# CPJKU/audio_sheet_retrieval

Hardware: AMD Instinct MI355X
Metric: snippet-pairs/sec embedded+ranked (32-d CCA) (higher is better)
Workload: dtype f32

## Files before the change

### audio_sheet_retrieval_amd/csrc/conv_wino4_kernels.hip

```cpp
#include <hip/hip_runtime.h>
#include <stdint.h>
#include <stdlib.h>
#include <algorithm>
#include <type_traits>
#include <vector>
#include "asr_kernels.h"
#include "repack_elems.inl"

#ifndef ASR_WINO4_ABL
#define ASR_WINO4_ABL 0
#endif

namespace asr {

typedef float floatx4q __attribute__((ext_vector_type(4)));
typedef float float2q __attribute__((ext_vector_type(2)));

struct Wino4Args {
    const float *in, *wpk, *bnp;
    float *out;
    int N, H, W, OH, OW;
    int ty_img, tx_img;
    int coutp;
    int tiles;
    int total;
    double *stats;
    BnBwdFuse bf;
};

__device__ __forceinline__ float elu_fastq(float y) { return y > 0.0f ? y : __expf(y) - 1.0f; }

template <typename T> __device__ __forceinline__ T splatq(float c);
template <> __device__ __forceinline__ float2q splatq<float2q>(float c) { return float2q{c, c}; }
template <> __device__ __forceinline__ floatx4q splatq<floatx4q>(float c) { return floatx4q{c, c, c, c}; }
template <typename T> __device__ __forceinline__ T fmaq(float c, T x, T y) {
    return __builtin_elementwise_fma(splatq<T>(c), x, y);
}

template <typename T> __device__ __forceinline__ void in6(T &d0, T &d1, T &d2, T &d3, T &d4, T &d5) {
    const T r0 = fmaq(4.f, d0, fmaq(-5.f, d2, d4));
    const T t1 = fmaq(-4.f, d2, d4), t2 = fmaq(-4.f, d1, d3);
    const T t3 = d4 - d2, t4 = d3 - d1;
    const T r5 = fmaq(4.f, d1, fmaq(-5.f, d3, d5));
    d0 = r0; d1 = t1 + t2; d2 = t1 - t2; d3 = fmaq(2.f, t4, t3); d4 = fmaq(-2.f, t4, t3); d5 = r5;
}
template <typename T> __device__ __forceinline__ void out6(T m0, T m1, T m2, T m3, T m4, T m5, T &y0, T &y1, T &y2, T &y3) {
    const T s1 = m1 + m2, s2 = m1 - m2, s3 = m3 + m4, s4 = m3 - m4;
    y0 = (m0 + s1) + s3;
    y1 = fmaq(2.f, s4, s2);
    y2 = fmaq(4.f, s3, s1);
    y3 = fmaq(8.f, s4, s2) + m5;
}

template <int CIN, int COUT, bool POOL, int WAVES, bool RAW>
__global__ __launch_bounds__(64 * WAVES, 1) void conv3x3_wino4g(Wino4Args a) {
    constexpr int KS = CIN / 4, NB = CIN / 8, T = 64 * WAVES;
    constexpr int WS = 16;
    constexpr int WD = 6;
    constexpr int WQ = 72;
    static_assert(CIN % 8 == 0, "channel blocks of 8");
    extern __shared__ __align__(16) float w_lds[];
    const int tid = threadIdx.x, lane = tid & 63;
    const int wave = __builtin_amdgcn_readfirstlane(tid >> 6);
    const int nt0 = blockIdx.y;
    for (int i = tid; i < KS * 36 * 4 * 16; i += T) {
        const int row = i >> 4, nn = i & 15;
        const int gg = row & 3, kp = row >> 2, ks = kp / 36, p = kp - ks * 36;
        const int qq = (ks & 1) * 36 + p;
        w_lds[i] = a.wpk[((((size_t)(ks >> 1) * 18 + (qq >> 2)) * 4 + gg) * a.coutp + nt0 * 16 + nn) * 4 + (qq & 3)];
    }
    __syncthreads();

    const int m = lane & 15, g = lane >> 4, n = lane & 15;
    const float *w_lane = w_lds + g * WS + n;
    const int chn = nt0 * 16 + n;
    const bool ch_ok = chn < COUT;
    const float bmean = (!RAW && ch_ok) ? a.bnp[chn] : 0.f;
    const float bscale = (!RAW && ch_ok) ? a.bnp[a.coutp + chn] : 1.f;
    const float bbeta = (!RAW && ch_ok) ? a.bnp[2 * a.coutp + chn] : 0.f;
    const int per_img = a.ty_img * a.tx_img;

    for (int mt = blockIdx.x * WAVES + wave; mt < a.total; mt += gridDim.x * WAVES) {
        const int tnum = mt * 16 + m;
        const bool tvalid = tnum < a.tiles;
        const int tcl = min(tnum, a.tiles - 1);
        const int img = tcl / per_img;
        const int trest = tcl - img * per_img;
        const int tty = trest / a.tx_img, ttx = trest - tty * a.tx_img;
        const int py = 4 * tty, px = 4 * ttx;
        const float *ibase = a.in + (int64_t)img * a.H * a.W * CIN + 2 * g;
        int rowb[6], colb[6];
        unsigned oy_m = 0, ox_m = 0;
#pragma unroll
        for (int i = 0; i < 6; ++i) {
            const int y = py - 1 + i, x = px - 1 + i;
            oy_m |= (unsigned)(y >= 0 && y < a.H) << i;
            ox_m |= (unsigned)(x >= 0 && x < a.W) << i;
            rowb[i] = min(max(y, 0), a.H - 1) * a.W * CIN;
            colb[i] = min(max(x, 0), a.W - 1) * CIN;
        }
        if (!tvalid) oy_m = 0;
        const bool interior = __builtin_amdgcn_ballot_w64(oy_m != 0x3fu || ox_m != 0x3fu) == 0;
        unsigned my_off;
        int my_ext;
        if (POOL) {
            my_off = (((unsigned)img * a.OH + 2 * tty) * a.OW + 2 * ttx) * COUT;
            const int nr = min(2, a.OH - 2 * tty), nc = min(2, a.OW - 2 * ttx);
            my_ext = (tvalid && nr > 0 && nc > 0) ? (nr | (nc << 8)) : 0;
        } else {
            my_off = (((unsigned)img * a.H + py) * a.W + px) * COUT;
            const int nr = min(4, a.H - py), nc = min(4, a.W - px);
            my_ext = tvalid ? (nr | (nc << 8)) : 0;
        }

        floatx4q acc[36];
#pragma unroll
        for (int p = 0; p < 36; ++p) acc[p] = floatx4q{0.f, 0.f, 0.f, 0.f};

        float2q nxt[6][6];
#pragma unroll
        for (int i = 0; i < 6; ++i)
#pragma unroll
            for (int j = 0; j < 6; ++j) nxt[i][j] = *reinterpret_cast<const float2q *>(ibase + rowb[i] + colb[j]);
        float wpre[WD];
#pragma unroll
        for (int q = 0; q < WD; ++q) wpre[q] = w_lane[q * 4 * WS];
#pragma unroll 1
        for (int t = 0; t < NB; ++t) {
            float2q dp[6][6];
            if (interior) {
#pragma unroll
                for (int i = 0; i < 6; ++i)
#pragma unroll
                    for (int j = 0; j < 6; ++j) dp[i][j] = nxt[i][j];
            } else {
#pragma unroll
                for (int i = 0; i < 6; ++i)
#pragma unroll
                    for (int j = 0; j < 6; ++j)
                        dp[i][j] = (((oy_m >> i) & (ox_m >> j)) & 1u) ? nxt[i][j] : float2q{0.f, 0.f};
            }
            if (t + 1 < NB && !(ASR_WINO4_ABL & 2)) {
#pragma unroll
                for (int i = 0; i < 6; ++i)
#pragma unroll
                    for (int j = 0; j < 6; ++j)
                        nxt[i][j] = *reinterpret_cast<const float2q *>(ibase + rowb[i] + colb[j] + 8 * (t + 1));
            }
#pragma unroll
            for (int j = 0; j < 6; ++j) in6(dp[0][j], dp[1][j], dp[2][j], dp[3][j], dp[4][j], dp[5][j]);
#pragma unroll
            for (int i = 0; i < 6; ++i) in6(dp[i][0], dp[i][1], dp[i][2], dp[i][3], dp[i][4], dp[i][5]);
            const float *wk = w_lane + (2 * t) * (36 * 4 * WS);
            const float *wn = (t + 1 < NB) ? wk + 2 * 36 * 4 * WS : w_lane;
            float wv[WQ + WD];
#pragma unroll
            for (int q = 0; q < WD; ++q) wv[q] = wpre[q];
#pragma unroll
            for (int q0 = 0; q0 < WQ; q0 += 2) {
#pragma unroll
                for (int q = q0; q < q0 + 2; ++q)
                    wv[q + WD] = (q + WD < WQ) ? wk[(q + WD) * 4 * WS] : wn[(q + WD - WQ) * 4 * WS];
                __builtin_amdgcn_sched_barrier(0);
#pragma unroll
                for (int q = q0; q < q0 + 2; ++q) {
                    const int c = q / 36, p = q % 36;
                    acc[p] = __builtin_amdgcn_mfma_f32_16x16x4f32(dp[p / 6][p % 6][c], wv[q], acc[p], 0, 0, 0);
                }
                __builtin_amdgcn_sched_barrier(0);
            }
#pragma unroll
            for (int q = 0; q < WD; ++q) wpre[q] = wv[WQ + q];
        }

        unsigned eo[4];
        int ee[4];
#pragma unroll
        for (int r = 0; r < 4; ++r) {
            eo[r] = (unsigned)__shfl((int)my_off, 4 * g + r);
            ee[r] = __shfl(my_ext, 4 * g + r);
        }
        if (!ch_ok) continue;
        floatx4q tc[4][6];
#pragma unroll
        for (int nu = 0; nu < 6; ++nu)
            out6(acc[nu], acc[6 + nu], acc[12 + nu], acc[18 + nu], acc[24 + nu], acc[30 + nu], tc[0][nu], tc[1][nu], tc[2][nu],
                 tc[3][nu]);
        if (POOL) {
#pragma unroll
            for (int pr = 0; pr < 2; ++pr) {
                floatx4q ya[4], yb[4];
                out6(tc[2 * pr][0], tc[2 * pr][1], tc[2 * pr][2], tc[2 * pr][3], tc[2 * pr][4], tc[2 * pr][5], ya[0], ya[1],
                     ya[2], ya[3]);
                out6(tc[2 * pr + 1][0], tc[2 * pr + 1][1], tc[2 * pr + 1][2], tc[2 * pr + 1][3], tc[2 * pr + 1][4],
                     tc[2 * pr + 1][5], yb[0], yb[1], yb[2], yb[3]);
#pragma unroll
                for (int pc = 0; pc < 2; ++pc) {
#pragma unroll
                    for (int r = 0; r < 4; ++r) {
                        if (pr >= (ee[r] & 0xff) || pc >= (ee[r] >> 8)) continue;
                        const float v0 = ya[2 * pc][r], v1 = ya[2 * pc + 1][r], v2 = yb[2 * pc][r], v3 = yb[2 * pc + 1][r];
                        const float hi = fmaxf(fmaxf(v0, v1), fmaxf(v2, v3));
                        const float lo = fminf(fminf(v0, v1), fminf(v2, v3));
                        const float x = bscale >= 0.0f ? hi : lo;
                        a.out[(size_t)eo[r] + (size_t)(pr * a.OW + pc) * COUT + chn] =
                            elu_fastq((x - bmean) * bscale + bbeta);
                    }
                }
            }
        } else {
#pragma unroll
            for (int i = 0; i < 4; ++i) {
                floatx4q y[4];
                out6(tc[i][0], tc[i][1], tc[i][2], tc[i][3], tc[i][4], tc[i][5], y[0], y[1], y[2], y[3]);
#pragma unroll
                for (int j = 0; j < 4; ++j) {
#pragma unroll
                    for (int r = 0; r < 4; ++r) {
                        if (i >= (ee[r] & 0xff) || j >= (ee[r] >> 8)) continue;
                        const float v = RAW ? y[j][r] : elu_fastq((y[j][r] - bmean) * bscale + bbeta);
                        a.out[(size_t)eo[r] + (size_t)(i * a.W + j) * COUT + chn] = v;
                    }
                }
            }
        }
    }
}

template <int CIN, int COUT, bool POOL, int SLICE = COUT, int PW = 1, bool RAW = false>
__global__ __launch_bounds__(64 * (PW + (SLICE + 15) / 16), 1) void conv3x3_wino4s(Wino4Args a) {
    static_assert(!(RAW && POOL), "the raw form has no pooled epilogue");
    constexpr int NT = (SLICE + 15) / 16, NB = CIN / 8, KS = CIN / 4;
    static_assert(PW == 1 || PW == 2, "one or two producer waves");
    static_assert(PW + NT <= 4, "one wave per SIMD");
    static_assert(SLICE == COUT || (SLICE % 16 == 0 && COUT % SLICE == 0), "slices are whole n-tiles");
    constexpr int VB = 36 * 16 * 8;
    static_assert(CIN % 8 == 0, "channel blocks of 8");
    extern __shared__ __align__(16) float vbuf[];
    const int tid = threadIdx.x, lane = tid & 63;
    const int wave = __builtin_amdgcn_readfirstlane(tid >> 6);
    const bool producer = wave < PW;
    const int m = lane & 15, g = lane >> 4, n = lane & 15;
    const int per_img = a.ty_img * a.tx_img;

    int mt, mt_end, mt_stride;
    if ((gridDim.x & 7) == 0) {
        const int per_x = (a.total + 7) >> 3;
        const int r0 = (int)(blockIdx.x & 7) * per_x;
        mt_end = min(r0 + per_x, a.total);
        mt_stride = (int)(gridDim.x >> 3);
        mt = r0 + (int)(blockIdx.x >> 3);
    } else {
        mt_end = a.total; mt_stride = (int)gridDim.x; mt = (int)blockIdx.x;
    }
    if (mt >= mt_end) {
        if constexpr (RAW) {
            if (a.stats)
                for (int c = threadIdx.x; c < 2 * COUT; c += blockDim.x) a.stats[(size_t)blockIdx.x * 2 * COUT + c] = 0.0;
        }
        return;
    }

    auto tile_of = [&](int mtile, int &img, int &tty, int &ttx, bool &tvalid) {
        const int tnum = mtile * 16 + m;
        tvalid = tnum < a.tiles;
        const int tcl = min(tnum, a.tiles - 1);
        img = tcl / per_img;
        const int trest = tcl - img * per_img;
        tty = trest / a.tx_img;
        ttx = trest - tty * a.tx_img;
    };
    float *vlane = vbuf + (g * 32 + 2 * m);
#ifdef ASR_WINO4_OLD_V
    vlane = vbuf + (m * 8 + 2 * g);
#endif

    if (producer) {
        unsigned poff[6][6];
        unsigned oy_m = 0, ox_m = 0;
        auto setup = [&](int mtile) {
            int img, tty, ttx;
            bool tvalid;
            tile_of(mtile, img, tty, ttx, tvalid);
            const int py = 4 * tty, px = 4 * ttx;
            const unsigned ib = ((unsigned)img * a.H * a.W * CIN + 2 * g) * 4u;
            unsigned rowb[6], colb[6];
            oy_m = 0; ox_m = 0;
#pragma unroll
            for (int i = 0; i < 6; ++i) {
                const int y = py - 1 + i, x = px - 1 + i;
                oy_m |= (unsigned)(y >= 0 && y < a.H) << i;
                ox_m |= (unsigned)(x >= 0 && x < a.W) << i;
                rowb[i] = (unsigned)(min(max(y, 0), a.H - 1) * a.W * CIN) * 4u;
                colb[i] = (unsigned)(min(max(x, 0), a.W - 1) * CIN) * 4u;
            }
            if (!tvalid) oy_m = 0;
#pragma unroll
            for (int i = 0; i < 6; ++i)
#pragma unroll
                for (int j = 0; j < 6; ++j) poff[i][j] = ib + rowb[i] + colb[j];
        };
        float2q nxt[6][6];
        auto load = [&](int t) {
            const char *cb = reinterpret_cast<const char *>(a.in + 8 * t);
#pragma unroll
            for (int i = 0; i < 6; ++i)
#pragma unroll
                for (int j = 0; j < 6; ++j) nxt[i][j] = *reinterpret_cast<const float2q *>(cb + poff[i][j]);
        };
        const int n_mt = (mt_end - mt + mt_stride - 1) / mt_stride;
        const int n_steps = n_mt * NB;
        int passed = 0;
        int t = wave;
        while (t >= NB) { t -= NB; mt += mt_stride; }
        if (mt < mt_end) { setup(mt); load(t); }
        for (int step = wave; step < n_steps; step += PW) {
            float2q dp[6][6];
            const unsigned oy = oy_m, ox = ox_m;
            const bool interior = __builtin_amdgcn_ballot_w64(oy != 0x3fu || ox != 0x3fu) == 0;
            if (interior) {
#pragma unroll
                for (int i = 0; i < 6; ++i)
#pragma unroll
                    for (int j = 0; j < 6; ++j) dp[i][j] = nxt[i][j];
            } else {
#pragma unroll
                for (int i = 0; i < 6; ++i)
#pragma unroll
                    for (int j = 0; j < 6; ++j) dp[i][j] = (((oy >> i) & (ox >> j)) & 1u) ? nxt[i][j] : float2q{0.f, 0.f};
            }
            {
                int tn = t + PW, mtn = mt;
                while (tn >= NB) { tn -= NB; mtn += mt_stride; }
                if (!(ASR_WINO4_ABL & 2) && step + PW < n_steps) {
                    if (mtn != mt) setup(mtn);
                    load(tn);
                }
                t = tn; mt = mtn;
            }
            if (!(ASR_WINO4_ABL & 8)) {
#pragma unroll
            for (int j = 0; j < 6; ++j) in6(dp[0][j], dp[1][j], dp[2][j], dp[3][j], dp[4][j], dp[5][j]);
#pragma unroll
            for (int i = 0; i < 6; ++i) in6(dp[i][0], dp[i][1], dp[i][2], dp[i][3], dp[i][4], dp[i][5]);
            }
            while (passed < step) { __syncthreads(); ++passed; }
            float *vb = vlane + (step & 1) * VB;
            if (!(ASR_WINO4_ABL & 16)) {
#pragma unroll
            for (int p = 0; p < 36; ++p) *reinterpret_cast<float2q *>(vb + p * 128) = dp[p / 6][p % 6];
            } else {
#pragma unroll
            for (int p = 0; p < 36; ++p) asm volatile("" ::"v"(dp[p / 6][p % 6]));
            }
            __syncthreads();
            ++passed;
        }
        while (passed < n_steps + 1) { __syncthreads(); ++passed; }
        return;
    }

    const int nt = wave - PW;
    const int chn = (int)blockIdx.y * SLICE + nt * 16 + n;
    const bool ch_ok = chn < COUT;
    float bmean = (!RAW && ch_ok) ? a.bnp[chn] : 0.f;
    float bscale = (!RAW && ch_ok) ? a.bnp[a.coutp + chn] : 1.f;
    float bbeta = (!RAW && ch_ok) ? a.bnp[2 * a.coutp + chn] : 0.f;
    float bistd = 0.f;
    const bool bnb = ASR_BNB_FUSE_BUILD && RAW && a.stats && a.bf.z != nullptr;
    if (bnb && ch_ok) {
        bmean = a.bf.cst[chn]; bistd = a.bf.cst[COUT + chn];
        bscale = a.bf.cst[2 * COUT + chn]; bbeta = a.bf.cst[3 * COUT + chn];
    }
    double st1 = 0.0, st2 = 0.0;
    const unsigned wlane = ((unsigned)g * a.coutp + chn) * 16u;
    const float *wl = a.wpk;
    constexpr int wstep = 4 * ((COUT + 15) / 16 * 16);
    floatx4q bw[2][18];
#pragma unroll
    for (int j = 0; j < 18; ++j)
        bw[0][j] = *reinterpret_cast<const floatx4q *>(reinterpret_cast<const char *>(wl) + (size_t)j * (wstep * 16) + wlane);
    int step = 0;
    for (; mt < mt_end; mt += mt_stride) {
        unsigned my_off;
        int my_ext;
        {
            int img, tty, ttx;
            bool tvalid;
            tile_of(mt, img, tty, ttx, tvalid);
            if (POOL) {
                my_off = (((unsigned)img * a.OH + 2 * tty) * a.OW + 2 * ttx) * COUT;
                const int nr = min(2, a.OH - 2 * tty), nc = min(2, a.OW - 2 * ttx);
                my_ext = (tvalid && nr > 0 && nc > 0) ? (nr | (nc << 8)) : 0;
            } else {
                my_off = (((unsigned)img * a.H + 4 * tty) * a.W + 4 * ttx) * COUT;
                const int nr = min(4, a.H - 4 * tty), nc = min(4, a.W - 4 * ttx);
                my_ext = tvalid ? (nr | (nc << 8)) : 0;
            }
        }
        unsigned voff[9];
#pragma unroll
        for (int k = 0; k < 9; ++k) {
            voff[k] = wlane + (unsigned)k * (2 * wstep * 16);
            asm volatile("" : "+v"(voff[k]));
        }
        floatx4q acc[36];
        auto reload = [&](const float *wn, auto set_c) {
            constexpr int SET = decltype(set_c)::value;
            if (ASR_WINO4_ABL & 4) return;
            const char *wnb = reinterpret_cast<const char *>(wn);
#pragma unroll
            for (int k = 0; k < 9; ++k) {
                unsigned vo = voff[k];
                asm volatile("" : "+v"(vo));
                bw[SET][2 * k] = *reinterpret_cast<const floatx4q *>(wnb + vo);
                bw[SET][2 * k + 1] = *reinterpret_cast<const floatx4q *>(wnb + (wstep * 16) + vo);
            }
        };
        auto run_step = [&](const float *vb, const float *wn, auto cur_c, auto first) {
            constexpr bool FIRST = decltype(first)::value;
            constexpr int CUR = decltype(cur_c)::value;
            using NXT = std::integral_constant<int, CUR ^ 1>;
            __syncthreads();
            reload(wn, NXT{});
            __builtin_amdgcn_sched_barrier(0);
            float2q dp[2][12];
#pragma unroll
            for (int i = 0; i < 12; ++i) dp[0][i] = *reinterpret_cast<const float2q *>(vb + i * 128);
#pragma unroll
            for (int grp = 0; grp < 3; ++grp) {
                if (grp < 2) {
#pragma unroll
                    for (int i = 0; i < 12; ++i)
                        dp[(grp + 1) & 1][i] = *reinterpret_cast<const float2q *>(vb + ((grp + 1) * 12 + i) * 128);
                }
#pragma unroll
                for (int c = 0; c < 2; ++c)
#pragma unroll
                    for (int i = 0; i < 12; ++i) {
                        const int p = grp * 12 + i;
                        if (FIRST && c == 0)
                            acc[p] = __builtin_amdgcn_mfma_f32_16x16x4f32(dp[grp & 1][i][c], bw[CUR][(c * 36 + p) >> 2][(c * 36 + p) & 3],
                                                                          floatx4q{0.f, 0.f, 0.f, 0.f}, 0, 0, 0);
                        else
                            acc[p] = __builtin_amdgcn_mfma_f32_16x16x4f32(dp[grp & 1][i][c], bw[CUR][(c * 36 + p) >> 2][(c * 36 + p) & 3], acc[p],
                                                                          0, 0,
                                                                          0);
                    }
                __builtin_amdgcn_sched_barrier(0);
            }
        };
        using C0 = std::integral_constant<int, 0>;
        using C1 = std::integral_constant<int, 1>;
        auto wblock = [&](int t) {
            unsigned blk = (unsigned)(((t + 1) % NB) * 72) * wstep;
            asm volatile("" : "+s"(blk));
            return wl + blk;
        };
        run_step(vlane + (step & 1) * VB, wblock(0), C0{}, std::true_type{});
        ++step;
#pragma unroll 1
        for (int t = 1; t + 1 < NB; t += 2) {
            run_step(vlane + (step & 1) * VB, wblock(t), C1{}, std::false_type{});
            ++step;
            run_step(vlane + (step & 1) * VB, wblock(t + 1), C0{}, std::false_type{});
            ++step;
        }
        if constexpr ((NB & 1) == 0) {
            run_step(vlane + (step & 1) * VB, wblock(NB - 1), C1{}, std::false_type{});
            ++step;
        } else {
#pragma unroll
            for (int j = 0; j < 18; ++j) bw[0][j] = bw[1][j];
        }

        unsigned eo[4];
        int ee[4];
#pragma unroll
        for (int r = 0; r < 4; ++r) {
            eo[r] = (unsigned)__shfl((int)my_off, 4 * g + r);
            ee[r] = __shfl(my_ext, 4 * g + r);
        }
        if (!ch_ok) continue;
        floatx4q tc[4][6];
#pragma unroll
        for (int nu = 0; nu < 6; ++nu)
            out6(acc[nu], acc[6 + nu], acc[12 + nu], acc[18 + nu], acc[24 + nu], acc[30 + nu], tc[0][nu], tc[1][nu], tc[2][nu],
                 tc[3][nu]);
        if (POOL) {
#pragma unroll
            for (int pr = 0; pr < 2; ++pr) {
                floatx4q ya[4], yb[4];
                out6(tc[2 * pr][0], tc[2 * pr][1], tc[2 * pr][2], tc[2 * pr][3], tc[2 * pr][4], tc[2 * pr][5], ya[0], ya[1],
                     ya[2], ya[3]);
                out6(tc[2 * pr + 1][0], tc[2 * pr + 1][1], tc[2 * pr + 1][2], tc[2 * pr + 1][3], tc[2 * pr + 1][4],
                     tc[2 * pr + 1][5], yb[0], yb[1], yb[2], yb[3]);
#pragma unroll
                for (int pc = 0; pc < 2; ++pc) {
#pragma unroll
                    for (int r = 0; r < 4; ++r) {
                        if (pr >= (ee[r] & 0xff) || pc >= (ee[r] >> 8)) continue;
                        const float v0 = ya[2 * pc][r], v1 = ya[2 * pc + 1][r], v2 = yb[2 * pc][r], v3 = yb[2 * pc + 1][r];
                        const float hi = fmaxf(fmaxf(v0, v1), fmaxf(v2, v3));
                        const float lo = fminf(fminf(v0, v1), fminf(v2, v3));
                        const float x = bscale >= 0.0f ? hi : lo;
                        const float res = elu_fastq((x - bmean) * bscale + bbeta);
                        if (ASR_WINO4_ABL & 32) asm volatile("" ::"v"(res));
                        else a.out[(size_t)eo[r] + (size_t)(pr * a.OW + pc) * COUT + chn] = res;
                    }
                }
            }
        } else {
#pragma unroll
            for (int i = 0; i < 4; ++i) {
                floatx4q y[4];
                out6(tc[i][0], tc[i][1], tc[i][2], tc[i][3], tc[i][4], tc[i][5], y[0], y[1], y[2], y[3]);
                float rs1 = 0.f, rs2 = 0.f;
#pragma unroll
                for (int j = 0; j < 4; ++j) {
#pragma unroll
                    for (int r = 0; r < 4; ++r) {
                        if (i >= (ee[r] & 0xff) || j >= (ee[r] >> 8)) continue;
                        const float res = RAW ? y[j][r] : elu_fastq((y[j][r] - bmean) * bscale + bbeta);
                        if (RAW) {
                            if (bnb) {
                                const size_t e = (size_t)eo[r] + (size_t)(i * a.W + j) * COUT + chn;
                                bnb_acc(res, a.bf.z[e], bnb_mult(a.bf.tie, e), bmean, bscale, bbeta, bistd, rs1, rs2);
                            } else { rs1 += res; rs2 = fmaf(res, res, rs2); }
                        }
                        if (ASR_WINO4_ABL & 32) asm volatile("" ::"v"(res));
                        else a.out[(size_t)eo[r] + (size_t)(i * a.W + j) * COUT + chn] = res;
                    }
                }
                if (RAW) { st1 += (double)rs1; st2 += (double)rs2; }
            }
        }
    }
    __syncthreads();
    if constexpr (RAW) {
        if (a.stats) {
            st1 += __shfl_xor(st1, 16); st2 += __shfl_xor(st2, 16);
            st1 += __shfl_xor(st1, 32); st2 += __shfl_xor(st2, 32);
            if (g == 0 && ch_ok) {
                a.stats[((size_t)blockIdx.x * 2) * COUT + chn] = st1;
                a.stats[((size_t)blockIdx.x * 2 + 1) * COUT + chn] = st2;
            }
        }
    }
}

__global__ void wino4_pack_kernel(const float *W, int cin, int cout, int dgrad, float *wpk) {
    const int idx = blockIdx.x * blockDim.x + threadIdx.x;
    if (idx >= wino4_pack_count(cin, cout, dgrad)) return;
    wino4_pack_elem(idx, W, cin, cout, dgrad, wpk);
}

size_t wino4_wpack_floats(int cin, int cout) { return (cin % 8) ? 0 : (size_t)36 * cin * ((cout + 15) / 16 * 16); }

hipError_t launch_wino4_pack(hipStream_t s, const float *W, int cin, int cout, float *wpk, int dgrad) {
    const int kdim = dgrad ? cout : cin, ndim = dgrad ? cin : cout;
    if (kdim % 8) return hipSuccess;
    const int total = kdim * ((ndim + 15) / 16 * 16);
    hipLaunchKernelGGL(wino4_pack_kernel, dim3((total + 255) / 256), dim3(256), 0, s, W, cin, cout, dgrad, wpk);
    return hipGetLastError();
}

struct Wino4Variant {
    int cin, cout, pool, waves, raw;
    void (*kernel)(Wino4Args);
    const char *symbol;
    int spec;
    int slice;
};
#define ASR_BOOLSTRQ_0 "false"
#define ASR_BOOLSTRQ_1 "true"
#define ASR_WINO4(CIN, COUT, POOL, WAVES)                                                                         \
    { CIN, COUT, POOL, WAVES, 0, conv3x3_wino4g<CIN, COUT, (POOL != 0), WAVES, false>,                            \
      "void asr::conv3x3_wino4g<" #CIN ", " #COUT ", " ASR_BOOLSTRQ_##POOL ", " #WAVES ", false>(asr::Wino4Args)" }
#define ASR_WINO4S(CIN, COUT, POOL)                                                                               \
    { CIN, COUT, POOL, 1 + (COUT + 15) / 16, 0, conv3x3_wino4s<CIN, COUT, (POOL != 0)>,                           \
      "void asr::conv3x3_wino4s<" #CIN ", " #COUT ", " ASR_BOOLSTRQ_##POOL ", " #COUT ", 1, false>(asr::Wino4Args)", 1, 0 }
#define ASR_WINO4S2(CIN, COUT, POOL)                                                                              \
    { CIN, COUT, POOL, 2 + (COUT + 15) / 16, 0, conv3x3_wino4s<CIN, COUT, (POOL != 0), COUT, 2>,                  \
      "void asr::conv3x3_wino4s<" #CIN ", " #COUT ", " ASR_BOOLSTRQ_##POOL ", " #COUT ", 2, false>(asr::Wino4Args)", 1, 0 }
#define ASR_WINO4SR(CIN, COUT)                                                                                    \
    { CIN, COUT, 0, 1 + (COUT + 15) / 16, 1, conv3x3_wino4s<CIN, COUT, false, COUT, 1, true>,                     \
      "void asr::conv3x3_wino4s<" #CIN ", " #COUT ", false, " #COUT ", 1, true>(asr::Wino4Args)", 1, 0 }
#define ASR_WINO4SL(CIN, COUT, POOL, SLICE)                                                                       \
    { CIN, COUT, POOL, 1 + SLICE / 16, 0, conv3x3_wino4s<CIN, COUT, (POOL != 0), SLICE>,                          \
      "void asr::conv3x3_wino4s<" #CIN ", " #COUT ", " ASR_BOOLSTRQ_##POOL ", " #SLICE ", 1, false>(asr::Wino4Args)", 1, SLICE }
static const Wino4Variant g_wino4[] = {
    ASR_WINO4(24, 24, 1, 4), ASR_WINO4(24, 48, 0, 4), ASR_WINO4(48, 48, 1, 4), ASR_WINO4(48, 48, 0, 4),
    ASR_WINO4S(24, 24, 1), ASR_WINO4S(24, 48, 0), ASR_WINO4S(48, 48, 1), ASR_WINO4S(48, 48, 0),
    ASR_WINO4S2(24, 24, 1),
    ASR_WINO4SL(48, 96, 0, 48), ASR_WINO4SL(96, 96, 1, 48), ASR_WINO4SL(96, 96, 0, 48),
    ASR_WINO4SR(24, 48), ASR_WINO4SR(48, 48), ASR_WINO4SR(48, 24),
};
static const int g_num_wino4 = (int)(sizeof(g_wino4) / sizeof(g_wino4[0]));

void conv_candidates_wino4(int cin, int cout, int pool, int H, int W, std::vector<ConvPlan> *out) {
    static const int use = getenv("ASR_CONV_WINO4") ? atoi(getenv("ASR_CONV_WINO4")) : -1;
    if (use == 0) return;
    for (int vi = 0; vi < g_num_wino4; ++vi) {
        const Wino4Variant &v = g_wino4[vi];
        if (v.cin != cin || v.cout != cout || v.pool != pool || v.raw) continue;
        if (!v.spec && use != 1) continue;
        const int lds = v.spec ? 2 * 36 * 16 * 8 * 4 : 36 * cin * 16 * 4;
        (void)hipFuncSetAttribute(reinterpret_cast<const void *>(v.kernel), hipFuncAttributeMaxDynamicSharedMemorySize,
                                  160 * 1024);
        int nb = 0;
        if (hipOccupancyMaxActiveBlocksPerMultiprocessor(&nb, reinterpret_cast<const void *>(v.kernel), 64 * v.waves,
                                                         (size_t)lds) != hipSuccess || nb < 1) {
            (void)hipGetLastError();
            nb = 1;
        }
        ConvPlan bp{};
        bp.cin = cin; bp.cout = cout; bp.pool = pool;
        bp.H = H; bp.W = W; bp.OH = pool ? H / 2 : H; bp.OW = pool ? W / 2 : W;
        bp.TH = 4; bp.TW = 64; bp.NI = 16;
        bp.tiles_y = (H + 3) / 4; bp.tiles_x = (W + 3) / 4;
        bp.threads = 64 * v.waves;
        bp.lds_bytes = lds;
        bp.blocks_per_cu = v.spec ? 1 : std::min(nb, 4);
        bp.cost = (double)bp.tiles_y * bp.tiles_x / 16.0 * ((cout + 15) / 16) * (36.0 * (cin / 4) * 32.0 + 3000.0) *
                  (v.spec ? 0.4 : 1.0);
        bp.variant = 4000 + vi;
        bp.symbol = v.symbol;
        out->push_back(bp);
    }
}

void conv_candidates_wino4_raw(int cin, int cout, int H, int W, std::vector<ConvPlan> *out, int dgrad) {
    static const int use = getenv("ASR_TRAIN_WINO4") ? atoi(getenv("ASR_TRAIN_WINO4")) : -1;
    if (use == 0 || (use == 5 && !dgrad)) return;
    for (int vi = 0; vi < g_num_wino4; ++vi) {
        const Wino4Variant &v = g_wino4[vi];
        if (v.cin != cin || v.cout != cout || !v.raw) continue;
        const int lds = 2 * 36 * 16 * 8 * 4;
        (void)hipFuncSetAttribute(reinterpret_cast<const void *>(v.kernel), hipFuncAttributeMaxDynamicSharedMemorySize,
                                  160 * 1024);
        ConvPlan bp{};
        bp.cin = cin; bp.cout = cout; bp.pool = 0;
        bp.H = H; bp.W = W; bp.OH = H; bp.OW = W;
        bp.TH = 4; bp.TW = 64; bp.NI = 16;
        bp.tiles_y = (H + 3) / 4; bp.tiles_x = (W + 3) / 4;
        bp.threads = 64 * v.waves;
        bp.lds_bytes = lds;
        bp.blocks_per_cu = 1;
        bp.cost = (double)bp.tiles_y * bp.tiles_x / 16.0 * ((cout + 15) / 16) * (36.0 * (cin / 4) * 32.0 + 3000.0) * 0.4;
        bp.variant = 4000 + vi;
        bp.symbol = v.symbol;
        out->push_back(bp);
    }
}
bool conv_wino4_is_raw(const ConvPlan &p) { return p.variant >= 4000 && g_wino4[p.variant - 4000].raw != 0; }
int conv_wino4_stats_rows_max(int num_cus) { return num_cus; }

hipError_t launch_conv_wino4(hipStream_t s, const ConvPlan &p, const float *in, const float *wpk, const float *bnp,
                             float *out, int N, int num_cus, double *stats, int *stats_rows, bool stats_clean,
                             const BnBwdFuse *bf) {
    const Wino4Variant &v = g_wino4[p.variant - 4000];
    Wino4Args a;
    a.stats = nullptr;
    a.bf = BnBwdFuse{nullptr, nullptr, nullptr};
    a.in = in; a.wpk = wpk; a.bnp = bnp; a.out = out;
    a.N = N; a.H = p.H; a.W = p.W; a.OH = p.OH; a.OW = p.OW;
    a.ty_img = p.tiles_y; a.tx_img = p.tiles_x;
    a.coutp = (p.cout + 15) / 16 * 16;
    a.tiles = N * a.ty_img * a.tx_img;
    a.total = (a.tiles + 15) / 16;
    if (a.total == 0) return hipSuccess;
    if (v.spec) {
        if ((double)N * p.H * p.W * p.cin * 4.0 >= 4294967296.0) return hipErrorInvalidValue;
        const int slices = v.slice ? p.cout / v.slice : 1;
        int grid = std::min(a.total, std::max(1, num_cus * std::max(1, p.blocks_per_cu) / slices));
        if (grid >= 8) grid &= ~7;
        if (v.raw && stats) {
            a.stats = stats;
            if (bf) a.bf = *bf;
            (void)stats_clean;
            if (stats_rows) *stats_rows = grid;
        }
        hipLaunchKernelGGL(v.kernel, dim3(grid, slices), dim3(p.threads), p.lds_bytes, s, a);
        return hipGetLastError();
    }
    const int ntiles = a.coutp / 16;
    const int waves = p.threads / 64;
    const int slots = std::max(1, num_cus * std::max(1, p.blocks_per_cu) / ntiles);
    const int grid = std::min((a.total + waves - 1) / waves, slots);
    hipLaunchKernelGGL(v.kernel, dim3(grid, ntiles), dim3(p.threads), p.lds_bytes, s, a);
    return hipGetLastError();
}

}
```

Baseline: 290,900.

## Add ring-buffered producer/consumer Winograd conv variants with LDS flag sync

Adds a RING template parameter to the specialised Winograd F(4,3) conv kernel. With it, producer waves write transformed input tiles into a ring of three or more LDS buffers and signal through per-slot full/done counters, instead of double buffering guarded by block-wide __syncthreads. The goal is to let producers run several steps ahead of the MFMA consumer waves and remove barrier stalls. New ring variants are registered as extra autotuning candidates, and an env var can force them on or off. The cost is more LDS per block, spin-wait polling with a bounded timeout, and relaxed-atomic ordering that relies on explicit lgkmcnt waits.

```diff
diff --git a/audio_sheet_retrieval_amd/csrc/conv_wino4_kernels.hip b/audio_sheet_retrieval_amd/csrc/conv_wino4_kernels.hip
--- a/audio_sheet_retrieval_amd/csrc/conv_wino4_kernels.hip
+++ b/audio_sheet_retrieval_amd/csrc/conv_wino4_kernels.hip
@@ -50,6 +50,12 @@
     y1 = fmaq(2.f, s4, s2);
     y2 = fmaq(4.f, s3, s1);
     y3 = fmaq(8.f, s4, s2) + m5;
+}
+
+__device__ __forceinline__ void ring_wait(unsigned *w, unsigned v) {
+    for (int spin = 0; __hip_atomic_load(w, __ATOMIC_RELAXED, __HIP_MEMORY_SCOPE_WORKGROUP) < v && spin < (1 << 20); ++spin)
+        __builtin_amdgcn_s_sleep(1);
+    asm volatile("" ::: "memory");
 }
 
 template <int CIN, int COUT, bool POOL, int WAVES, bool RAW>
@@ -227,9 +233,10 @@
     }
 }
 
-template <int CIN, int COUT, bool POOL, int SLICE = COUT, int PW = 1, bool RAW = false>
+template <int CIN, int COUT, bool POOL, int SLICE = COUT, int PW = 1, int RING = 0, bool RAW = false>
 __global__ __launch_bounds__(64 * (PW + (SLICE + 15) / 16), 1) void conv3x3_wino4s(Wino4Args a) {
     static_assert(!(RAW && POOL), "the raw form has no pooled epilogue");
+    static_assert(RING == 0 || (RING >= 3 && !RAW), "ring of three buffers or more, inference builds");
     constexpr int NT = (SLICE + 15) / 16, NB = CIN / 8, KS = CIN / 4;
     static_assert(PW == 1 || PW == 2, "one or two producer waves");
     static_assert(PW + NT <= 4, "one wave per SIMD");
@@ -242,6 +249,8 @@
     const bool producer = wave < PW;
     const int m = lane & 15, g = lane >> 4, n = lane & 15;
     const int per_img = a.ty_img * a.tx_img;
+    unsigned *ring_full = reinterpret_cast<unsigned *>(vbuf + (RING ? RING : 2) * VB);
+    unsigned *ring_done = ring_full + RING;
 
     int mt, mt_end, mt_stride;
     if ((gridDim.x & 7) == 0) {
@@ -259,6 +268,10 @@
                 for (int c = threadIdx.x; c < 2 * COUT; c += blockDim.x) a.stats[(size_t)blockIdx.x * 2 * COUT + c] = 0.0;
         }
         return;
+    }
+    if constexpr (RING > 0) {
+        if (tid < 2 * RING) ring_full[tid] = 0u;
+        __syncthreads();
     }
 
     auto tile_of = [&](int mtile, int &img, int &tty, int &ttx, bool &tvalid) {
@@ -310,6 +323,53 @@
         };
         const int n_mt = (mt_end - mt + mt_stride - 1) / mt_stride;
         const int n_steps = n_mt * NB;
+        if constexpr (RING > 0) {
+            int t = wave;
+            while (t >= NB) { t -= NB; mt += mt_stride; }
+            if (mt < mt_end) { setup(mt); load(t); }
+            int r = wave, use = 0;
+            while (r >= RING) { r -= RING; ++use; }
+            for (int step = wave; step < n_steps; step += PW) {
+                float2q dp[6][6];
+                const unsigned oy = oy_m, ox = ox_m;
+                const bool interior = __builtin_amdgcn_ballot_w64(oy != 0x3fu || ox != 0x3fu) == 0;
+                if (interior) {
+#pragma unroll
+                    for (int i = 0; i < 6; ++i)
+#pragma unroll
+                        for (int j = 0; j < 6; ++j) dp[i][j] = nxt[i][j];
+                } else {
+#pragma unroll
+                    for (int i = 0; i < 6; ++i)
+#pragma unroll
+                        for (int j = 0; j < 6; ++j) dp[i][j] = (((oy >> i) & (ox >> j)) & 1u) ? nxt[i][j] : float2q{0.f, 0.f};
+                }
+                {
+                    int tn = t + PW, mtn = mt;
+                    while (tn >= NB) { tn -= NB; mtn += mt_stride; }
+                    if (!(ASR_WINO4_ABL & 2) && step + PW < n_steps) {
+                        if (mtn != mt) setup(mtn);
+                        load(tn);
+                    }
+                    t = tn; mt = mtn;
+                }
+                if (!(ASR_WINO4_ABL & 8)) {
+#pragma unroll
+                for (int j = 0; j < 6; ++j) in6(dp[0][j], dp[1][j], dp[2][j], dp[3][j], dp[4][j], dp[5][j]);
+#pragma unroll
+                for (int i = 0; i < 6; ++i) in6(dp[i][0], dp[i][1], dp[i][2], dp[i][3], dp[i][4], dp[i][5]);
+                }
+                ring_wait(ring_done + r, (unsigned)(NT * use));
+                float *vb = vlane + r * VB;
+#pragma unroll
+                for (int p = 0; p < 36; ++p) *reinterpret_cast<float2q *>(vb + p * 128) = dp[p / 6][p % 6];
+                asm volatile("s_waitcnt lgkmcnt(0)" ::: "memory");
+                if (lane == 0) __hip_atomic_store(ring_full + r, (unsigned)(step + 1), __ATOMIC_RELAXED, __HIP_MEMORY_SCOPE_WORKGROUP);
+                r += PW;
+                if (r >= RING) { r -= RING; ++use; }
+            }
+            return;
+        }
         int passed = 0;
         int t = wave;
         while (t >= NB) { t -= NB; mt += mt_stride; }
@@ -381,6 +441,7 @@
     for (int j = 0; j < 18; ++j)
         bw[0][j] = *reinterpret_cast<const floatx4q *>(reinterpret_cast<const char *>(wl) + (size_t)j * (wstep * 16) + wlane);
     int step = 0;
+    int ring_r = 0;
     for (; mt < mt_end; mt += mt_stride) {
         unsigned my_off;
         int my_ext;
@@ -421,7 +482,8 @@
             constexpr bool FIRST = decltype(first)::value;
             constexpr int CUR = decltype(cur_c)::value;
             using NXT = std::integral_constant<int, CUR ^ 1>;
-            __syncthreads();
+            if constexpr (RING > 0) ring_wait(ring_full + ring_r, (unsigned)(step + 1));
+            else __syncthreads();
             reload(wn, NXT{});
             __builtin_amdgcn_sched_barrier(0);
             float2q dp[2][12];
@@ -449,7 +511,13 @@
                     }
                 __builtin_amdgcn_sched_barrier(0);
             }
+            if constexpr (RING > 0) {
+                asm volatile("s_waitcnt lgkmcnt(0)" ::: "memory");
+                if (lane == 0) __hip_atomic_fetch_add(ring_done + ring_r, 1u, __ATOMIC_RELAXED, __HIP_MEMORY_SCOPE_WORKGROUP);
+                if (++ring_r == RING) ring_r = 0;
+            }
         };
+        auto vcur = [&]() { return vlane + (RING > 0 ? ring_r : (step & 1)) * VB; };
         using C0 = std::integral_constant<int, 0>;
         using C1 = std::integral_constant<int, 1>;
         auto wblock = [&](int t) {
@@ -457,17 +525,17 @@
             asm volatile("" : "+s"(blk));
             return wl + blk;
         };
-        run_step(vlane + (step & 1) * VB, wblock(0), C0{}, std::true_type{});
+        run_step(vcur(), wblock(0), C0{}, std::true_type{});
         ++step;
 #pragma unroll 1
         for (int t = 1; t + 1 < NB; t += 2) {
-            run_step(vlane + (step & 1) * VB, wblock(t), C1{}, std::false_type{});
+            run_step(vcur(), wblock(t), C1{}, std::false_type{});
             ++step;
-            run_step(vlane + (step & 1) * VB, wblock(t + 1), C0{}, std::false_type{});
+            run_step(vcur(), wblock(t + 1), C0{}, std::false_type{});
             ++step;
         }
         if constexpr ((NB & 1) == 0) {
-            run_step(vlane + (step & 1) * VB, wblock(NB - 1), C1{}, std::false_type{});
+            run_step(vcur(), wblock(NB - 1), C1{}, std::false_type{});
             ++step;
         } else {
 #pragma unroll
@@ -536,6 +604,7 @@
             }
         }
     }
+    if constexpr (RING > 0) return;
     __syncthreads();
     if constexpr (RAW) {
         if (a.stats) {
@@ -571,7 +640,9 @@
     const char *symbol;
     int spec;
     int slice;
+    int ring;
 };
+static int wino4s_lds_bytes(int ring) { return ring ? ring * (36 * 16 * 8 * 4) + 2 * ring * 4 : 2 * 36 * 16 * 8 * 4; }
 #define ASR_BOOLSTRQ_0 "false"
 #define ASR_BOOLSTRQ_1 "true"
 #define ASR_WINO4(CIN, COUT, POOL, WAVES)                                                                         \
@@ -579,33 +650,50 @@
       "void asr::conv3x3_wino4g<" #CIN ", " #COUT ", " ASR_BOOLSTRQ_##POOL ", " #WAVES ", false>(asr::Wino4Args)" }
 #define ASR_WINO4S(CIN, COUT, POOL)                                                                               \
     { CIN, COUT, POOL, 1 + (COUT + 15) / 16, 0, conv3x3_wino4s<CIN, COUT, (POOL != 0)>,                           \
-      "void asr::conv3x3_wino4s<" #CIN ", " #COUT ", " ASR_BOOLSTRQ_##POOL ", " #COUT ", 1, false>(asr::Wino4Args)", 1, 0 }
+      "void asr::conv3x3_wino4s<" #CIN ", " #COUT ", " ASR_BOOLSTRQ_##POOL ", " #COUT ", 1, 0, false>(asr::Wino4Args)", 1, 0, 0 }
 #define ASR_WINO4S2(CIN, COUT, POOL)                                                                              \
     { CIN, COUT, POOL, 2 + (COUT + 15) / 16, 0, conv3x3_wino4s<CIN, COUT, (POOL != 0), COUT, 2>,                  \
-      "void asr::conv3x3_wino4s<" #CIN ", " #COUT ", " ASR_BOOLSTRQ_##POOL ", " #COUT ", 2, false>(asr::Wino4Args)", 1, 0 }
+      "void asr::conv3x3_wino4s<" #CIN ", " #COUT ", " ASR_BOOLSTRQ_##POOL ", " #COUT ", 2, 0, false>(asr::Wino4Args)", 1, 0, 0 }
 #define ASR_WINO4SR(CIN, COUT)                                                                                    \
-    { CIN, COUT, 0, 1 + (COUT + 15) / 16, 1, conv3x3_wino4s<CIN, COUT, false, COUT, 1, true>,                     \
-      "void asr::conv3x3_wino4s<" #CIN ", " #COUT ", false, " #COUT ", 1, true>(asr::Wino4Args)", 1, 0 }
+    { CIN, COUT, 0, 1 + (COUT + 15) / 16, 1, conv3x3_wino4s<CIN, COUT, false, COUT, 1, 0, true>,                  \
+      "void asr::conv3x3_wino4s<" #CIN ", " #COUT ", false, " #COUT ", 1, 0, true>(asr::Wino4Args)", 1, 0, 0 }
 #define ASR_WINO4SL(CIN, COUT, POOL, SLICE)                                                                       \
     { CIN, COUT, POOL, 1 + SLICE / 16, 0, conv3x3_wino4s<CIN, COUT, (POOL != 0), SLICE>,                          \
-      "void asr::conv3x3_wino4s<" #CIN ", " #COUT ", " ASR_BOOLSTRQ_##POOL ", " #SLICE ", 1, false>(asr::Wino4Args)", 1, SLICE }
+      "void asr::conv3x3_wino4s<" #CIN ", " #COUT ", " ASR_BOOLSTRQ_##POOL ", " #SLICE ", 1, 0, false>(asr::Wino4Args)", 1, SLICE, 0 }
+#define ASR_WINO4SQ(CIN, COUT, POOL, PW, R)                                                                       \
+    { CIN, COUT, POOL, PW + (COUT + 15) / 16, 0, conv3x3_wino4s<CIN, COUT, (POOL != 0), COUT, PW, R>,             \
+      "void asr::conv3x3_wino4s<" #CIN ", " #COUT ", " ASR_BOOLSTRQ_##POOL ", " #COUT ", " #PW ", " #R ", false>(asr::Wino4Args)", \
+      1, 0, R }
 static const Wino4Variant g_wino4[] = {
     ASR_WINO4(24, 24, 1, 4), ASR_WINO4(24, 48, 0, 4), ASR_WINO4(48, 48, 1, 4), ASR_WINO4(48, 48, 0, 4),
     ASR_WINO4S(24, 24, 1), ASR_WINO4S(24, 48, 0), ASR_WINO4S(48, 48, 1), ASR_WINO4S(48, 48, 0),
     ASR_WINO4S2(24, 24, 1),
     ASR_WINO4SL(48, 96, 0, 48), ASR_WINO4SL(96, 96, 1, 48), ASR_WINO4SL(96, 96, 0, 48),
     ASR_WINO4SR(24, 48), ASR_WINO4SR(48, 48), ASR_WINO4SR(48, 24),
+    ASR_WINO4SQ(24, 48, 0, 1, 4), ASR_WINO4SQ(48, 48, 1, 1, 4), ASR_WINO4SQ(48, 48, 0, 1, 4), ASR_WINO4SQ(24, 24, 1, 1, 4),
+    ASR_WINO4SQ(24, 24, 1, 2, 4),
 };
 static const int g_num_wino4 = (int)(sizeof(g_wino4) / sizeof(g_wino4[0]));
 
 void conv_candidates_wino4(int cin, int cout, int pool, int H, int W, std::vector<ConvPlan> *out) {
     static const int use = getenv("ASR_CONV_WINO4") ? atoi(getenv("ASR_CONV_WINO4")) : -1;
+    static const int ring = getenv("ASR_WINO4_RING") ? atoi(getenv("ASR_WINO4_RING")) : -1;
     if (use == 0) return;
     for (int vi = 0; vi < g_num_wino4; ++vi) {
         const Wino4Variant &v = g_wino4[vi];
         if (v.cin != cin || v.cout != cout || v.pool != pool || v.raw) continue;
         if (!v.spec && use != 1) continue;
-        const int lds = v.spec ? 2 * 36 * 16 * 8 * 4 : 36 * cin * 16 * 4;
+        if (ring == 0 && v.ring) continue;
+        if (ring == 1 && v.spec && !v.ring) {
+            bool has_ring = false;
+            for (int wi = 0; wi < g_num_wino4; ++wi) {
+                const Wino4Variant &w = g_wino4[wi];
+                has_ring = has_ring || (w.ring && w.cin == v.cin && w.cout == v.cout && w.pool == v.pool &&
+                                        w.waves == v.waves && w.slice == v.slice);
+            }
+            if (has_ring) continue;
+        }
+        const int lds = v.spec ? wino4s_lds_bytes(v.ring) : 36 * cin * 16 * 4;
         (void)hipFuncSetAttribute(reinterpret_cast<const void *>(v.kernel), hipFuncAttributeMaxDynamicSharedMemorySize,
                                   160 * 1024);
         int nb = 0;
```

Measured after the change: 294,400, median of 6. +1.2%, better.
